# NBDsoftware/deep_cartograph

Measured on AMD Instinct MI355X. Metric: Deep-TICA training frames/sec on 10Mx512 feature matrix at 1/2/4/8 GPUs, higher is better.
Workload: dtype f32

## Files before the change

deep_cartograph_amd/csrc/gemm.h:

```cpp
#pragma once
#include <type_traits>
#include "common.h"
#include "handoff.h"

namespace dcv {

#ifdef DCV_STAMP
__device__ unsigned long long g_stamp[8 * 8192];
#define DCV_STAMP_AT(slot)                                                                      \
    do {                                                                                        \
        if (threadIdx.x == 0 && blockIdx.x < 8192 && blockIdx.z == 0)                           \
            g_stamp[blockIdx.x * 8 + (slot)] = __builtin_amdgcn_s_memtime();                   \
    } while (0)
#define DCV_STAMP_RT(slot)                                                                      \
    do {                                                                                        \
        if (threadIdx.x == 0 && blockIdx.x < 8192 && blockIdx.z == 0)                           \
            g_stamp[blockIdx.x * 8 + (slot)] = __builtin_amdgcn_s_memrealtime();               \
    } while (0)
#else
#define DCV_STAMP_AT(slot) do {} while (0)
#define DCV_STAMP_RT(slot) do {} while (0)
#endif

typedef float f32x16 __attribute__((ext_vector_type(16)));
// ... 43 lines not shown
    const float* p;
    int64_t ld;
    RowMap rows;
    const float* shift;
    int vec_ok;
    int planes = 0;
    int64_t pstride = 0;
};

struct GemmDims {
    int64_t M, N, K;
    int64_t k_chunk;
    int tiles_m, tiles_n;
    int xcd_remap;
    int wt;
    int tail_split = 0;
    float* tail_ws = nullptr;
    unsigned* tail_cnt = nullptr;
};

template <int WAVES_M_, int WAVES_N_, int FM_, int FN_, int KB_, int NBUF_ = 2, bool SPLIT_ = false, int PL_ = 0>
struct TileCfg {
    static constexpr int WAVES_M = WAVES_M_, WAVES_N = WAVES_N_, FM = FM_, FN = FN_, KB = KB_, NBUF = NBUF_;
    static constexpr bool SPLIT = SPLIT_;
    static constexpr int PL = PL_;
    static_assert(PL == 0 || SPLIT, "plane operands belong to the split flavour");
    static constexpr bool LS = (PL_ & 16) != 0;
    static constexpr int RAW_SZ = LS ? (WAVES_M_ * FM_ * 32 + WAVES_N_ * FN_ * 32) * KB_ : 0;
    static constexpr int A_SZ = (PL & 5) ? 3 * (WAVES_M_ * FM_ * 32) * (KB_ / 2) : (WAVES_M_ * FM_ * 32) * KB_;
    static constexpr int B_SZ = (PL & 10) ? 3 * (WAVES_N_ * FN_ * 32) * (KB_ / 2) : (WAVES_N_ * FN_ * 32) * KB_;
    static_assert(NBUF >= 2 && NBUF <= 8, "NBUF");
    static constexpr int TM = WAVES_M * FM * 32;
    static constexpr int TN = WAVES_N * FN * 32;
    static_assert(WAVES_M * WAVES_N == 4, "4 waves per workgroup");
    static_assert(KB == 16 || KB == 32, "KB");
};

template <int KB>
__device__ __forceinline__ int mmajor_off(int row, int chunk) {
    constexpr int CPR = KB / 4;
    constexpr int RPBR = 64 / KB;
    return row * KB + ((chunk ^ ((row / RPBR) % CPR)) << 2);
}

__device__ __forceinline__ void glds16(const float* gsrc, unsigned lds_wave_addr) {
    unsigned keep;
    asm volatile(
        "s_mov_b32 %0, m0\n\t"
        "s_mov_b32 m0, %2\n\t"
        "s_nop 0\n\t"
        "global_load_lds_dwordx4 %1, off\n\t"
        "s_mov_b32 m0, %0"
        : "=&s"(keep)
        : "v"(gsrc), "s"(lds_wave_addr)
        : "memory");
}
__device__ __forceinline__ unsigned lds_addr_uniform(const float* p) {
    const unsigned a = (unsigned)(uintptr_t)(__attribute__((address_space(3))) const float*)p;
    return __builtin_amdgcn_readfirstlane(a);
}

template <int PER>
__device__ __forceinline__ void glds16_batch(const float* base, const unsigned (&voff)[PER], unsigned lds0) {
    static_assert(PER == 1 || PER == 2 || PER == 4, "units per thread");
    unsigned keep;
    if constexpr (PER == 1) {
        asm volatile(
            "s_mov_b32 %0, m0\n\ts_nop 3\n\t"
// ... 296 lines not shown
__device__ __forceinline__ void vm_wait_younger(int64_t younger) {
    if constexpr (MAXY == 0) vm_wait<EXTRA>();
    else {
        if (younger >= MAXY) vm_wait<MAXY * GL + EXTRA>();
        else vm_wait_younger<MAXY - 1, GL, EXTRA>(younger);
    }
}

template <int MODE, class Cfg, int NB, bool VEC, bool GATHER, class Epi>
__device__ __forceinline__ void gemm_block(const Operand& A, const Operand& B, int64_t lag2, const GemmDims& d,
                                           int tile_m, int tile_n, int64_t k_begin, int64_t k_end, float* lds,
                                           Epi& epi, int tail_chunk = -1) {
    constexpr int TM = Cfg::TM, TN = Cfg::TN, KB = Cfg::KB, FM = Cfg::FM, FN = Cfg::FN;
    constexpr int A_SZ = Cfg::A_SZ, B_SZ = Cfg::B_SZ;
    constexpr int STAGE = A_SZ + NB * B_SZ;
    constexpr bool A_MM = (MODE == kNT || MODE == kNN);
    constexpr bool B_MM = (MODE == kNT);
    constexpr int PL = Cfg::PL;
    constexpr bool PRE = (PL & 3) != 0;
    constexpr bool PSA = (PL & 4) != 0, PSB = (PL & 8) != 0;
    constexpr bool PA = (PL & 5) != 0, PB = (PL & 10) != 0;
    constexpr bool LS = Cfg::LS;
    static_assert(!LS || (MODE == kNT && PSA && PSB && VEC && !GATHER && NB == 1), "split-from-LDS: NT products, both operands, 16-byte rows");
    static_assert(!PRE || (MODE == kNT && NB == 1 && VEC && Cfg::SPLIT), "plane operands: NT products of the split flavour");
    static_assert(!(PSA || PSB) || (!PRE && NB == 1 && Cfg::SPLIT), "split-at-store: split flavour, one B operand, no pre-split operand beside it");
    static_assert(!PSA || MODE == kNT || MODE == kNN, "split-at-store of A needs a contraction-contiguous A");
    static_assert(!PSB || MODE == kNT, "split-at-store of B needs a contraction-contiguous B");
    constexpr int KF = KB / 2;
    constexpr int KA = (PL & 1) ? KF : KB, KBB = (PL & 2) ? KF : KB;
    constexpr int NPA = (PL & 1) ? 3 : 1, NPB = (PL & 2) ? 3 : 1;
    const int t = threadIdx.x;
    const int lane = t & 63;
    const int wave = t >> 6;
    const int wm = (wave / Cfg::WAVES_N) * FM * 32;
    const int wn = (wave % Cfg::WAVES_N) * FN * 32;
    const int64_t m0 = (int64_t)tile_m * TM, n0 = (int64_t)tile_n * TN;
#ifdef DCV_ABL_SAMETILE
    const int64_t m0_ld = (int64_t)(tile_m % DCV_ABL_SAMETILE) * TM;
#else
    const int64_t m0_ld = m0;
#endif

    f32x16 acc[NB][FM][FN];
#pragma unroll
    for (int b = 0; b < NB; ++b)
#pragma unroll
        for (int i = 0; i < FM; ++i)
#pragma unroll
            for (int j = 0; j < FN; ++j)
#pragma unroll
                for (int e = 0; e < 16; ++e) acc[b][i][j][e] = 0.f;

    MMajorStage<TM, KA, VEC, GATHER> am;
    KMajorStage<TM, KB, VEC, GATHER> ak;
    MMajorStage<TN, KBB, VEC, GATHER> bm;
    KMajorStage<TN, KB, VEC, GATHER> bk[NB];
    if constexpr (A_MM) am.template init<PRE || LS>(A, m0, d.M, t);
    else ak.init(A, m0, d.M, t);
    if constexpr (B_MM) bm.template init<PRE || LS>(B, n0, d.N, t);
    else {
#pragma unroll
        for (int b = 0; b < NB; ++b) bk[b].init(B, n0, d.N, t);
    }

    auto resolve_stage = [&](int64_t k0) {
        if constexpr (!A_MM) ak.resolve(A, k0, k_end, 0, t);
        if constexpr (!B_MM) {
            bk[0].resolve(B, k0, k_end, 0, t);
// ... 292 lines not shown
        if constexpr (kASum) {
#pragma unroll
            for (int i = 0; i < FM; ++i) asum[i] += (f.a[i][0] + f.a[i][1]) + (f.a[i][2] + f.a[i][3]);
        }
    };
    auto mfma_step = [&](const Frags& f, int s) {
#pragma unroll
        for (int b = 0; b < NB; ++b)
#pragma unroll
            for (int i = 0; i < FM; ++i)
#pragma unroll
                for (int j = 0; j < FN; ++j)
                    acc[b][i][j] = __builtin_amdgcn_mfma_f32_32x32x2f32(f.a[i][s], f.b[b][j][s], acc[b][i][j], 0, 0, 0);
    };
    auto mfma_group = [&](const Frags& f) {
#pragma unroll
        for (int s = 0; s < 4; ++s)
#pragma unroll
            for (int b = 0; b < NB; ++b)
#pragma unroll
                for (int i = 0; i < FM; ++i)
#pragma unroll
                    for (int j = 0; j < FN; ++j)
                        acc[b][i][j] = __builtin_amdgcn_mfma_f32_32x32x2f32(f.a[i][s], f.b[b][j][s], acc[b][i][j], 0, 0, 0);
    };

    const int64_t nst = (k_end - k_begin + KB - 1) / KB;
    DCV_STAMP_AT(0);
#ifdef DCV_STAMP
    if (threadIdx.x == 0 && blockIdx.x < 8192 && blockIdx.z == 0)
        g_stamp[blockIdx.x * 8 + 7] = (unsigned long long)__builtin_amdgcn_s_getreg(63492) | ((unsigned long long)__builtin_amdgcn_s_getreg(63508) << 32);
#endif
    constexpr int G = KB / 8;
    auto compute_stage = [&](const float* cur) {
        const float* la = cur;
        const float* lb = cur + A_SZ;
        if constexpr (Cfg::SPLIT) {
#pragma unroll
            for (int s = 0; s < KB / 16; ++s) {
                Frags8 f;
                read_frags8(f, la, lb, s);
                mfma16(f);
            }
            return;
        }
#ifndef DCV_NO_FRAG_DBUF
        Frags f0, f1;
        read_frags(f0, la, lb, 0);
#pragma unroll
        for (int g = 0; g < G; g += 2) {
            if (g + 1 < G) read_frags(f1, la, lb, g + 1);
            add_asum(f0);
            mfma_group(f0);
            if (g + 1 < G) {
                if (g + 2 < G) read_frags(f0, la, lb, g + 2);
                add_asum(f1);
                mfma_group(f1);
            }
        }
#else
#pragma unroll
        for (int g = 0; g < G; ++g) {
            Frags f0;
            read_frags(f0, la, lb, g);
            add_asum(f0);
            mfma_group(f0);
        }
#endif
    };
// ... 62 lines not shown
    if (nfull > 0) {
        const int64_t nst = nfull;
        constexpr int NBUF = Cfg::NBUF;
        constexpr int GL = (A_MM ? NPA * MMajorStage<TM, KA, VEC, GATHER>::PER : KMajorStage<TM, KB, VEC, GATHER>::PER) +
                           NB * (B_MM ? NPB * MMajorStage<TN, KBB, VEC, GATHER>::PER : KMajorStage<TN, KB, VEC, GATHER>::PER);
        static_assert((NBUF - 2) * GL <= 63, "vmcnt range");
        static_assert(Cfg::SPLIT || G % 2 == 0, "fragment double buffer parity");
#pragma unroll
        for (int s = 0; s < NBUF - 1; ++s)
            if (s < nst) glds_stage(k_begin + s * KB, s);
        if constexpr (kSidePre) {
            static_assert((NBUF - 2) * GL + EPASS * ENQ <= 63, "vmcnt range");
            side_ready = epi.vec && (m0 + TM <= d.M) && (n0 + TN <= d.N);
            if constexpr (Epi::kMaskIn) side_ready = side_ready && epi.mask == nullptr;
            if (side_ready) {
                const int ec4 = t % EC4, er0 = t / EC4;
#pragma unroll
                for (int q = 0; q < EPASS * ENQ; ++q)
                    side_pre[q] = *reinterpret_cast<const float4*>(epi.side_ptr(m0 + er0 + q * ERPP, n0 + ec4 * 4));
                vm_wait_younger<NBUF - 2, GL, EPASS * ENQ>(nst - 1);
            } else {
                vm_wait_younger<NBUF - 2, GL>(nst - 1);
            }
        } else {
            vm_wait_younger<NBUF - 2, GL>(nst - 1);
        }
        __syncthreads();
#ifndef DCV_ABL_NOLOAD
        if (NBUF - 1 < nst) glds_stage(k_begin + (NBUF - 1) * KB, NBUF - 1);
#endif
        DCV_STAMP_AT(1);
        DCV_STAMP_RT(5);
        if constexpr (Cfg::SPLIT) {
            constexpr int S = KB / 16;
            Frags8 f0, f1;
#ifdef DCV_PIPE_SPLIT
            Planes pl0, pl1;
#endif
            read_frags8(f0, lds, lds + A_SZ, 0);
#ifdef DCV_PIPE_SPLIT
            if constexpr (S == 2) split_frags(f0, pl0);
#endif
            int cur_buf = 0;
            for (int64_t st = 0; st < nst; ++st) {
                const float* la = lds + cur_buf * STAGE;
                const float* lb = la + A_SZ;
                const int nxt_buf = cur_buf + 1 == NBUF ? 0 : cur_buf + 1;
#ifdef DCV_PIPE_SPLIT
                if constexpr (S == 2) {
                    constexpr int NMF = 6 * NB * FM * FN;
                    constexpr int NVA = 44 * (FM + NB * FN);
                    constexpr int VPM = (NVA + NMF - 1) / NMF;
                    read_frags8(f1, la, lb, 1);
                    mfma_planes(pl0, [](int) {});
                    split_frags(f1, pl1);
                    pin_planes(pl1);
#pragma unroll
                    for (int q = 0; q < NMF; ++q) {
                        __builtin_amdgcn_sched_group_barrier(0x008, 1, 0);
                        __builtin_amdgcn_sched_group_barrier(0x002, VPM, 0);
                    }
                    __builtin_amdgcn_sched_barrier(0);
                    vm_wait_younger<NBUF - 2, GL>(nst - 2 - st);
                    __syncthreads();
                    read_frags8(f0, lds + nxt_buf * STAGE, lds + nxt_buf * STAGE + A_SZ, 0);
                    const bool more = st + NBUF < nst;
                    const int64_t k_next = k_begin + (st + NBUF) * KB;
                    __builtin_amdgcn_sched_barrier(0);
                    if (more) glds_stage(k_next, cur_buf, 3);
                    __builtin_amdgcn_sched_barrier(0);
                    mfma_planes(pl1, [](int) {});
                    split_frags(f0, pl0);
// ... 5 lines not shown
                    }
                    __builtin_amdgcn_sched_barrier(0);
                } else
#endif
                if constexpr (S == 2) {
                    read_frags8(f1, la, lb, 1);
                    mfma16(f0);
                    Planes pl;
                    split_frags(f1, pl);
                    vm_wait_younger<NBUF - 2, GL>(nst - 2 - st);
#ifndef DCV_ABL_NOBARRIER
                    __syncthreads();
#endif
                    read_frags8(f0, lds + nxt_buf * STAGE, lds + nxt_buf * STAGE + A_SZ, 0);
                    const bool more = st + NBUF < nst;
                    const int64_t k_next = k_begin + (st + NBUF) * KB;
                    mfma_planes(pl, [&](int k) {
#ifndef DCV_ABL_NOLOAD
                        if (k == 0 || k == 2) {
                            __builtin_amdgcn_sched_barrier(0);
                            if (more) glds_stage(k_next, cur_buf, k == 0 ? 1 : 2);
                            __builtin_amdgcn_sched_barrier(0);
                        }
#endif
                    });
                } else {
                    vm_wait_younger<NBUF - 2, GL>(nst - 2 - st);
#ifndef DCV_ABL_NOBARRIER
                    __syncthreads();
#endif
#ifndef DCV_ABL_NOLOAD
                    if (st + NBUF < nst) glds_stage(k_begin + (st + NBUF) * KB, cur_buf);
#endif
                    read_frags8(f1, lds + nxt_buf * STAGE, lds + nxt_buf * STAGE + A_SZ, 0);
                    mfma16(f0);
                    f0 = f1;
                }
                cur_buf = nxt_buf;
            }
            __syncthreads();
        } else {
        Frags f0, f1;
        read_frags(f0, lds, lds + A_SZ, 0);
        int cur_buf = 0;
        for (int64_t st = 0; st < nst; ++st) {
            const float* la = lds + cur_buf * STAGE;
            const float* lb = la + A_SZ;
            const int nxt_buf = cur_buf + 1 == NBUF ? 0 : cur_buf + 1;
#pragma unroll
            for (int g = 0; g < G; g += 2) {
                read_frags(f1, la, lb, g + 1);
                __builtin_amdgcn_sched_barrier(0);
                pin_frags(f0);
                if (dma_sub) sub_frags(f0);
                add_asum(f0);
                mfma_group(f0);
                __builtin_amdgcn_sched_barrier(0);
                if (g + 2 < G) {
                    read_frags(f0, la, lb, g + 2);
                    __builtin_amdgcn_sched_barrier(0);
                    pin_frags(f1);
                    if (dma_sub) sub_frags(f1);
                    add_asum(f1);
                    mfma_group(f1);
                    __builtin_amdgcn_sched_barrier(0);
                } else {
                    vm_wait_younger<NBUF - 2, GL>(nst - 2 - st);
// ... 18 lines not shown
                    __builtin_amdgcn_sched_barrier(0);
                    mfma_step(f1, 2);
                    __builtin_amdgcn_sched_barrier(0);
                    read_frags(f0, lds + nxt_buf * STAGE, lds + nxt_buf * STAGE + A_SZ, 0);
                    __builtin_amdgcn_sched_barrier(0);
                    mfma_step(f1, 3);
                    __builtin_amdgcn_sched_barrier(0);
                }
            }
            cur_buf = nxt_buf;
        }
        __syncthreads();
        }
    } else {
        DCV_STAMP_AT(1);
        DCV_STAMP_RT(5);
    }
    const int64_t k_rem = k_begin + nfull * KB;
    const int64_t nrem = (PRE || LS) ? 0 : (k_end - k_rem + KB - 1) / KB;
    if (nrem > 0) {
        resolve_stage(k_rem);
        load_stage(k_rem);
        if (nrem > 1) resolve_stage(k_rem + KB);
        store_stage(lds);
        __syncthreads();
        for (int64_t st = 0; st < nrem; ++st) {
            const float* cur = lds + (st & 1) * STAGE;
            float* nxt = lds + ((st + 1) & 1) * STAGE;
            const bool more = st + 1 < nrem;
            if (more) {
                load_stage(k_rem + (st + 1) * KB);
                if (st + 2 < nrem) resolve_stage(k_rem + (st + 2) * KB);
            }
            if (MODE == kTN || m0 + wm < d.M) compute_stage(cur);
            if (more) store_stage(nxt);
            __syncthreads();
        }
    }
    if constexpr (MODE != kTN && NB == 1) {
        if (tail_chunk >= 0) {
            constexpr int NACC = FM * FN * 16;
            const int S = d.tail_split;
            float* ws = d.tail_ws + (int64_t)tile_n * S * NACC * 256;
            float* mine = ws + (int64_t)tail_chunk * NACC * 256 + t;
#pragma unroll
            for (int i = 0; i < FM; ++i)
#pragma unroll
                for (int j = 0; j < FN; ++j)
#pragma unroll
                    for (int e = 0; e < 16; ++e) handoff_store(mine + ((i * FN + j) * 16 + e) * 256, acc[0][i][j][e]);
            const bool last = handoff_arrive_last(d.tail_cnt + tile_n, (unsigned)S, reinterpret_cast<unsigned*>(lds));
            __syncthreads();
            if (!last) return;
#pragma unroll
            for (int i = 0; i < FM; ++i)
#pragma unroll
                for (int j = 0; j < FN; ++j)
#pragma unroll
                    for (int e = 0; e < 16; ++e) acc[0][i][j][e] = 0.f;
            for (int c = 0; c < S; ++c) {
                const float* part = ws + (int64_t)c * NACC * 256 + t;
#pragma unroll
                for (int i = 0; i < FM; ++i)
#pragma unroll
                    for (int j = 0; j < FN; ++j)
#pragma unroll
                        for (int e = 0; e < 16; ++e) acc[0][i][j][e] += handoff_load(part + ((i * FN + j) * 16 + e) * 256);
            }
        }
    }
#ifdef DCV_ABL_NOEPI
    {
        float sink = 0.f;
#pragma unroll
        for (int b = 0; b < NB; ++b)
#pragma unroll
            for (int i = 0; i < FM; ++i)
#pragma unroll
                for (int j = 0; j < FN; ++j)
#pragma unroll
                    for (int e = 0; e < 16; ++e) sink += acc[b][i][j][e];
        if (sink != 12345.678f) return;
    }
#endif

    DCV_STAMP_AT(2);
    DCV_STAMP_RT(6);
    static_assert(!Epi::kHead || kStaged, "the fused narrow layer needs the staged epilogue");
    if constexpr (kStaged) {
        float* tile = lds;
        constexpr int C4 = TN / 4;
        constexpr int RPP = 256 / C4;
        constexpr int NQ = RP / RPP;
        const int c4 = t % C4, r0 = t / C4;
        const int64_t col = n0 + c4 * 4;
        const int64_t left = d.N - col;
        const int nvalid = left >= 4 ? 4 : (left > 0 ? (int)left : 0);
        const bool fast = epi.vec && (m0 + TM <= d.M) && (n0 + TN <= d.N);
        const float4 cc = nvalid > 0 ? epi.colconst(col, nvalid) : make_float4(0.f, 0.f, 0.f, 0.f);
        constexpr int EQ = NQ < 8 ? NQ : 8;
        static_assert(NQ % EQ == 0, "epilogue chunking");
        float4 cs = make_float4(0.f, 0.f, 0.f, 0.f);
#pragma unroll
        for (int ep = 0; ep < EPASS; ++ep) {
            if (ep > 0) __syncthreads();
            if (wm / RP == ep) {
#pragma unroll
                for (int i = 0; i < FM; ++i)
#pragma unroll
                    for (int j = 0; j < FN; ++j) {
                        const int c = wn + j * 32 + (lane & 31);
                        const int rb = wm - ep * RP + i * 32 + 4 * (lane >> 5);
#pragma unroll
                        for (int e = 0; e < 16; ++e) tile[(rb + (e & 3) + 8 * (e >> 2)) * TN + c] = acc[0][i][j][e];
                    }
            }
            __syncthreads();
            if (ep == 0) DCV_STAMP_AT(3);
            const int64_t mbase = m0 + ep * RP;
#pragma unroll
            for (int qc = 0; qc < NQ; qc += EQ) {
                float4 v[EQ], side[Epi::kSide ? EQ : 1];
// ... 115 lines not shown
```

deep_cartograph_amd/csrc/gemm.hip:

```cpp
#include <type_traits>
#include "gemm_kernels.h"

using namespace dcv;

namespace dcv {
int gemm_nn_store(const Operand& A, const Operand& B, int64_t M, int64_t N, int64_t K, const EpiStore& epi, hipStream_t s) {
    return launch_gemm<kNN, EpiStore>(A, B, M, N, K, 0, epi, s);
}
}

extern "C" int dcv_gemm_f32(int32_t mode, const float* A_d, int64_t lda, const float* B_d, int64_t ldb, float* C_d,
                            int64_t ldc, int64_t M, int64_t N, int64_t K, void* stream) {
    DCV_REQUIRE(A_d && B_d && C_d && M > 0 && N > 0 && K > 0, "dcv_gemm_f32: bad arguments");
    hipStream_t s = as_stream(stream);
    const Operand A = make_operand(A_d, lda, 0);
    const Operand B = make_operand(B_d, ldb, 0);
    EpiStore epi{C_d, ldc, quad_ok(C_d, ldc)};
    switch (mode) {
        case kNT: return launch_gemm<kNT, EpiStore>(A, B, M, N, K, 0, epi, s);
        case kNN: return gemm_nn_store(A, B, M, N, K, epi, s);
        case kTN: return launch_gemm<kTN, EpiStore>(A, B, M, N, K, 0, epi, s);
        default: set_error("dcv_gemm_f32: mode %d", mode); return DCV_EINVAL;
    }
}

extern "C" int dcv_gemm_tn_split(const float* A_d, int64_t lda, const float* B_d, int64_t ldb, float* slab_d, int64_t slab_cap,
                                 int64_t M, int64_t N, int64_t K, int64_t k_chunk, void* stream) {
    DCV_REQUIRE(A_d && B_d && slab_d && M > 0 && N > 0 && K > 0 && k_chunk > 0 && slab_cap > 0, "dcv_gemm_tn_split: bad arguments");
    const Operand A = make_operand(A_d, lda, 0);
    const Operand B = make_operand(B_d, ldb, 0);
    EpiSlab epi{slab_d, M, N, 1, 0, quad_ok(slab_d, N), slab_cap};
    return gemm_tn_slab(A, B, M, N, K, k_chunk, epi, as_stream(stream));
}
```

deep_cartograph_amd/csrc/gemm_kernels.h:

```cpp
#pragma once
#include <type_traits>
#include <stdlib.h>
#include <hip/hip_ext.h>
#include "gemm.h"

namespace dcv {

constexpr float kSoftplus0 = 0.6931471824645996f;
__device__ __forceinline__ float act_fwd(int act, float z) {
    switch (act) {
        case DCV_ACT_LEAKY_RELU: return z > 0.f ? z : 0.01f * z;
        case DCV_ACT_RELU: return z > 0.f ? z : 0.f;
        case DCV_ACT_TANH: return tanhf(z);
        case DCV_ACT_ELU: return z > 0.f ? z : expm1f(z);
        case DCV_ACT_SOFTPLUS: return z > 20.f ? z : log1pf(expf(z));
        case DCV_ACT_SHIFTED_SOFTPLUS: return (z > 20.f ? z : log1pf(expf(z))) - kSoftplus0;
        case DCV_ACT_CUSTOM_SIGMOID: return 1.f / (1.f + expf(-3.f * z));
        default: return z;
    }
}
__device__ __forceinline__ float act_grad_from_out(int act, float h) {
    switch (act) {
        case DCV_ACT_LEAKY_RELU: return h > 0.f ? 1.f : 0.01f;
        case DCV_ACT_RELU: return h > 0.f ? 1.f : 0.f;
// ... 323 lines not shown
        gemm_block<kNN, Cfg2, 1, true, false, EpiActGrad>(A2, B2, 0, d2, bm.tile_m, bm.tile_n, bm.k_begin, bm.k_end, lds_f, e2, bm.tail_chunk);
    }
}

struct GroupShift {
    int64_t a_rows = 0;
    int64_t a_floats = 0;
    int64_t out_rows = 0;
    int64_t tail_floats = 0;
    int tail_tickets = 0;
};
template <class Cfg, bool VEC, bool GATHER, class Epi>
__global__ __launch_bounds__(256, 2) void gemm_group_kernel(Operand A, Operand B, GemmDims d, Epi epi, GroupShift g) {
    extern __shared__ __attribute__((aligned(16))) float lds_f[];
    const int64_t j = blockIdx.y;
    A.p += j * g.a_floats;
    if (A.rows.idx != nullptr) A.rows.idx += j * g.a_rows;
    else A.rows.row0 += j * g.a_rows;
    epi.shift_rows(j * g.out_rows);
    if (d.tail_split > 0) {
        d.tail_ws += j * g.tail_floats;
        d.tail_cnt += j * g.tail_tickets;
    }
    const BlockMap bm = map_block<kNT>(d, (int)blockIdx.x);
    gemm_block<kNT, Cfg, 1, VEC, GATHER, Epi>(A, B, 0, d, bm.tile_m, bm.tile_n, bm.k_begin, bm.k_end, lds_f, epi, bm.tail_chunk);
}

template <bool S> using CfgBigT = TileCfg<2, 2, 2, 2, 32, 2, S>;
template <bool S> using CfgHalfMT = TileCfg<2, 2, 1, 2, 32, 2, S>;
template <bool S> using CfgQuarterT = TileCfg<2, 2, 1, 1, 32, 2, S>;
template <bool S> using CfgNarrowNT = TileCfg<4, 1, 1, 1, 32, 2, S>;
template <bool S> using CfgNarrowMT = TileCfg<1, 4, 1, 1, 32, 2, S>;
template <bool S> using CfgCovT = TileCfg<2, 2, 2, 2, 16, 2, S>;
#ifdef DCV_BIGCFG
using CfgBig = DCV_BIGCFG;
#else
using CfgBig = CfgBigT<false>;
#endif

template <int MODE, class Cfg, int NB, bool VEC, bool GATHER, class Epi>
static int launch_gemm_vec(const Operand& A, const Operand& B, int64_t lag2, const GemmDims& d, int64_t splits,
                           const Epi& epi, hipStream_t s) {
#ifdef DCV_FORCE_LDS
    constexpr size_t lds = DCV_FORCE_LDS;
#else
    constexpr size_t lds = gemm_lds_bytes<Cfg, NB>();
#endif
    auto kern = gemm_kernel<MODE, Cfg, NB, VEC, GATHER, Epi>;
    if (lds > 64 * 1024) {
        static bool attr_set = false;
        if (!attr_set) {
            DCV_CHECK_HIP(hipFuncSetAttribute(reinterpret_cast<const void*>(kern), hipFuncAttributeMaxDynamicSharedMemorySize, (int)lds));
            attr_set = true;
        }
    }
    const int64_t blocks = d.tail_split > 0 ? (int64_t)(d.tiles_m - 1 + d.tail_split) * d.tiles_n : (int64_t)d.tiles_m * d.tiles_n;
    if (g_launch_ev.start != nullptr) {
        const LaunchEvents ev = g_launch_ev;
        g_launch_ev = LaunchEvents{};
        g_launch_taken = ev.start;
        hipExtLaunchKernelGGL(kern, dim3((unsigned)blocks, 1, (unsigned)splits), dim3(256), (uint32_t)lds, s, ev.start, ev.stop, 0u, A, B, lag2, d, epi);
    } else {
        hipLaunchKernelGGL(kern, dim3((unsigned)blocks, 1, (unsigned)splits), dim3(256), lds, s, A, B, lag2, d, epi);
    }
    DCV_CHECK_LAUNCH();
    return DCV_OK;
// ... 171 lines not shown
            }
        }
    }
#endif
#ifdef DCV_PS_EXPERIMENT
    if constexpr (S && MODE == kNT && !Epi::kHead) {
        static const bool ls_on = [] { const char* e = getenv("DCV_LS"); return e && e[0] == '1'; }();
        if (ls_on && pick == kPickQuarter) {
            const int rc = launch_gemm_ls<TileCfg<2, 2, 1, 1, 32, 2, true, 28>, Epi>(A, B, M, N, K, epi, s, tiles_m_out, tw);
            if (rc != 1) return rc;
        }
    }
#endif
    switch (pick) {
        case kPickNarrowN: return launch_gemm_cfg<MODE, CfgNarrowNT<S>, 1, Epi>(A, B, 0, M, N, K, k_chunk, epi, s, tiles_m_out, tw);
        case kPickNarrowM: return launch_gemm_cfg<MODE, CfgNarrowMT<S>, 1, Epi>(A, B, 0, M, N, K, k_chunk, epi, s, tiles_m_out, tw);
        case kPickHalfM: return launch_gemm_cfg<MODE, CfgHalfMT<S>, 1, Epi>(A, B, 0, M, N, K, k_chunk, epi, s, tiles_m_out, tw);
        case kPickQuarter:
            if constexpr (!Epi::kHead) return launch_gemm_cfg<MODE, CfgQuarterT<S>, 1, Epi>(A, B, 0, M, N, K, k_chunk, epi, s, tiles_m_out, tw);
            else return launch_gemm_cfg<MODE, CfgHalfMT<S>, 1, Epi>(A, B, 0, M, N, K, k_chunk, epi, s, tiles_m_out, tw);
        default: return launch_gemm_cfg<MODE, Big, 1, Epi>(A, B, 0, M, N, K, k_chunk, epi, s, tiles_m_out, tw);
    }
}

template <int MODE, class Epi>
static int launch_gemm(const Operand& A, const Operand& B, int64_t M, int64_t N, int64_t K, int64_t k_chunk,
                       const Epi& epi, hipStream_t s, int* tiles_m_out = nullptr, const TailWs* tw = nullptr) {
#ifdef DCV_BIGCFG
    return launch_gemm_mode<MODE, false, Epi>(A, B, M, N, K, k_chunk, epi, s, tiles_m_out, tw);
#else
    if (gemm_split()) return launch_gemm_mode<MODE, true, Epi>(A, B, M, N, K, k_chunk, epi, s, tiles_m_out, tw);
    return launch_gemm_mode<MODE, false, Epi>(A, B, M, N, K, k_chunk, epi, s, tiles_m_out, tw);
#endif
}

template <bool S, bool HEAD, class F>
static int with_cfg(CfgPick pick, F&& f) {
    switch (pick) {
        case kPickNarrowN: return f(CfgNarrowNT<S>{});
        case kPickNarrowM: return f(CfgNarrowMT<S>{});
        case kPickHalfM: return f(CfgHalfMT<S>{});
        case kPickQuarter:
            if constexpr (!HEAD) return f(CfgQuarterT<S>{});
            else return f(CfgHalfMT<S>{});
        default: return f(CfgBigT<S>{});
    }
}
inline bool group_retile_enabled() {
    static const bool on = [] { const char* e = getenv("DCV_EVAL_GROUP_TILES"); return !(e && e[0] == '0'); }();
    return on;
}
template <bool S, class Epi>
static int launch_gemm_group_mode(const Operand& A, const Operand& B, int64_t M, int64_t N, int64_t K, const Epi& epi, const GroupShift& g,
                                  int members, const TailWs* tw, hipStream_t s) {
    constexpr bool HEAD = Epi::kHead;
    DCV_REQUIRE(members >= 1 && members < 65536, "gemm: %d members in a grouped launch", members);
    const CfgPick pick1 = pick_cfg<kNT, HEAD>(M, N, K, 0);
    GemmPlan single;
    int64_t tm1 = 0;
    int rc = with_cfg<S, HEAD>(pick1, [&](auto c) {
        using C1 = decltype(c);
        tm1 = C1::TM;
        return prepare_gemm<kNT, C1, 1, Epi>(A, B, M, N, K, 0, epi, nullptr, tw, &single);
    });
    if (rc) return rc;
    if (!single.vec) return 1;
// ... 19 lines not shown
            if (r) return r;
            if (!pl.vec) return 1;
            if (single.d.tail_split > 0) {
                constexpr int64_t TM2 = C2::TM;
                const int64_t S1 = single.d.tail_split;
                if (M % TM2 == 0 || (M / TM2) * TM2 != (M / tm1) * tm1 || pl.d.tiles_m < 2 || K % C2::KB != 0) return 1;
                if (pl.d.tiles_n > tw->max_tiles_n || (int64_t)pl.d.tiles_n * S1 * C2::FM * C2::FN * 16 * 256 > tw->cap) return 1;
                pl.d.tail_split = (int)S1;
                pl.d.k_chunk = single.d.k_chunk;
                pl.d.tail_ws = single.d.tail_ws;
                pl.d.tail_cnt = single.d.tail_cnt;
                pl.d.xcd_remap = xcd_remap_enabled() && (pl.d.tiles_m - 1) % 8 == 0 && pl.d.tiles_n > 1;
            }
            return go(c, pl);
        });
        if (rc != 1) return rc;
    }
    return with_cfg<S, HEAD>(pick1, [&](auto c) { return go(c, single); });
}
template <class Epi>
static int launch_gemm_group(const Operand& A, const Operand& B, int64_t M, int64_t N, int64_t K, const Epi& epi, const GroupShift& g, int members,
                             const TailWs* tw, hipStream_t s) {
    if (gemm_split()) return launch_gemm_group_mode<true, Epi>(A, B, M, N, K, epi, g, members, tw, s);
    return launch_gemm_group_mode<false, Epi>(A, B, M, N, K, epi, g, members, tw, s);
}

int gemm_nt_bias_act(const Operand& A, const Operand& B, int64_t M, int64_t N, int64_t K, const EpiBiasAct& epi, hipStream_t s, const TailWs* tw);
int gemm_nt_head4(const Operand& A, const Operand& B, int64_t M, int64_t N, int64_t K, const EpiBiasActHead<4>& epi, hipStream_t s, const TailWs* tw);
int gemm_nt_head8(const Operand& A, const Operand& B, int64_t M, int64_t N, int64_t K, const EpiBiasActHead<8>& epi, hipStream_t s, const TailWs* tw);
int gemm_nt_bias_act_group(const Operand& A, const Operand& B, int64_t M, int64_t N, int64_t K, const EpiBiasAct& epi, const GroupShift& g, int members,
                           const TailWs* tw, hipStream_t s);
int gemm_nt_head4_group(const Operand& A, const Operand& B, int64_t M, int64_t N, int64_t K, const EpiBiasActHead<4>& epi, const GroupShift& g, int members,
                        const TailWs* tw, hipStream_t s);
int gemm_tn_slab(const Operand& A, const Operand& B, int64_t M, int64_t N, int64_t K, int64_t k_chunk, const EpiSlab& epi, hipStream_t s);
int gemm_nn_act_grad(const Operand& A, const Operand& B, int64_t M, int64_t N, int64_t K, const EpiActGrad& epi, hipStream_t s,
                     int* tiles_m_out, const TailWs* tw);
int gemm_nn_store(const Operand& A, const Operand& B, int64_t M, int64_t N, int64_t K, const EpiStore& epi, hipStream_t s);

int launch_wgrad_dgrad(const Operand& A1, const Operand& B1, int64_t M1, int64_t N1, int64_t K1, int64_t k_chunk1, const EpiSlab& e1,
                       const Operand& A2, const Operand& B2, int64_t M2, int64_t N2, int64_t K2, const EpiActGrad& e2, int* tiles_m_out2,
                       const TailWs* tw, hipStream_t s);

__host__ __device__ inline int64_t planes_kp(int64_t cols) { return (cols + 31) / 32 * 32; }
__host__ __device__ inline int64_t planes_ld(int64_t cols) { return 3 * planes_kp(cols) / 2; }
__host__ __device__ inline int64_t planes_pstride(int64_t cols) { return planes_kp(cols) / 2; }
inline size_t planes_bytes(int64_t rows, int64_t cols) { return (size_t)rows * (size_t)planes_ld(cols) * sizeof(float); }
template <bool TRANS>
__global__ __launch_bounds__(256) void split_planes_kernel(const float* __restrict__ src, int64_t ld, int64_t rows, int64_t cols,
                                                           float* __restrict__ dst, int64_t rows_out) {
    const int64_t orows = TRANS ? cols : rows, ocols = TRANS ? rows : cols;
    const int64_t kp8 = planes_kp(ocols) / 8, ldp = planes_ld(ocols), ps = planes_pstride(ocols);
    const int64_t total = rows_out * kp8;
    for (int64_t i = (int64_t)blockIdx.x * 256 + threadIdx.x; i < total; i += (int64_t)gridDim.x * 256) {
        const int64_t r = i / kp8, g = i - r * kp8;
        float x[8];
#pragma unroll
        for (int e = 0; e < 8; ++e) {
            const int64_t k = 8 * g + e;
            x[e] = (r < orows && k < ocols) ? (TRANS ? src[k * ld + r] : src[r * ld + k]) : 0.f;
        }
        u32x4 p1, p2, p3;
        split3(x, p1, p2, p3);
        float* o = dst + r * ldp + g * 4;
        *reinterpret_cast<u32x4*>(o) = p1;
        *reinterpret_cast<u32x4*>(o + ps) = p2;
        *reinterpret_cast<u32x4*>(o + 2 * ps) = p3;
    }
// ... 90 lines not shown
```

deep_cartograph_amd/csrc/inst_wgrad.hip:

```cpp
#include "gemm_kernels.h"

namespace dcv {

int gemm_tn_slab(const Operand& A, const Operand& B, int64_t M, int64_t N, int64_t K, int64_t k_chunk, const EpiSlab& epi, hipStream_t s) {
    return launch_gemm<kTN, EpiSlab>(A, B, M, N, K, k_chunk, epi, s);
}

}
```

deep_cartograph_amd/csrc/mlp.hip:

```cpp
#include "mlp_state.h"
#include "tica_head.h"
#include <new>
#include <math.h>

using namespace dcv;

namespace dcv {

constexpr int kColsumRows = 32;
constexpr int kSseRows = 16;
constexpr int kStatBlockRows = 128;

__global__ __launch_bounds__(256) void colsum_kernel(const float* __restrict__ Z, int64_t rows, int n, int64_t ld,
                                                     float* __restrict__ part) {
    __shared__ float red[256];
    const int64_t r0 = (int64_t)blockIdx.x * kColsumRows;
    const int64_t r1 = r0 + kColsumRows < rows ? r0 + kColsumRows : rows;
    const int t = threadIdx.x;
    const int cols = n < 256 ? n : 256;
    const int groups = 256 / cols;
    const int c_in = t % cols, g = t / cols;
    for (int c0 = 0; c0 < n; c0 += cols) {
        const int c = c0 + c_in;
        float s = 0.f;
// ... 2135 lines not shown
            prof_mark(m, l, 1, 1, s);
            Operand Bd = make_operand(m->params + p.w_off, p.in, p.in);
            EpiActGrad eg{dz_nxt, m->ld_dz, m->vae_z, m->ld_z, DCV_ACT_NONE, hd.bpart, p.in, quad_ok(dz_nxt, m->ld_dz) && quad_ok(m->vae_z, m->ld_z)};
            int dblocks = 0;
            prof_mark(m, l, 2, 0, s);
            rc = gemm_nn_act_grad(A, Bd, R, p.in, p.out, eg, s, &dblocks, &m->tail);
            if (rc) return rc;
            hipLaunchKernelGGL(vae_sample_backward_kernel, dim3((unsigned)cdiv(R, kVaeRows)), dim3(kVaeRows), 0, s, (const float*)hd.H, hd.ldh, R,
                               m->vae_d, m->eps_cur, dz_nxt, m->ld_dz, (float)(m->kl_beta / (double)global_batch));
            DCV_CHECK_LAUNCH();
            bblocks = (int)cdiv(R, kColsumRows);
            hipLaunchKernelGGL(colsum_kernel, dim3(bblocks), dim3(256), 0, s, (const float*)dz_nxt, R, hd.out, m->ld_dz, hd.bpart);
            DCV_CHECK_LAUNCH();
            prof_mark(m, l, 2, 1, s);
            float* tmp = dz_cur;
            dz_cur = dz_nxt;
            dz_nxt = tmp;
            continue;
        }
        Operand A = make_operand(dz_cur, m->ld_dz, p.out);
        Operand B = l == 0 ? make_operand(Xn_d, ld, p.in, rm) : make_operand(layer_out(m, l - 1), m->layers[l - 1].ldh, p.in);
        EpiSlab epi{p.slab, p.out, p.in, 1, 0, quad_ok(p.slab, p.in), p.max_splits};
        ReduceDesc& rd = ra.l[l];
        rd.slab = p.slab;
        rd.bpart = p.bpart;
        rd.w_off = p.w_off;
        rd.b_off = p.b_off;
        rd.w_count = (int64_t)p.out * p.in;
        rd.out = p.out;
        rd.splits = (int)splits;
        rd.bblocks = bblocks;
        if (l == 0) {
            prof_mark(m, l, 1, 0, s);
            int rc = gemm_tn_slab(A, B, p.out, p.in, R, kc, epi, s);
            if (rc) return rc;
            prof_mark(m, l, 1, 1, s);
            continue;
        }
        LayerPlan& q = m->layers[l - 1];
        Operand Ad = make_operand(dz_cur, m->ld_dz, p.out);
        Operand Bd = make_operand(m->params + p.w_off, p.in, p.in);
        EpiActGrad eg{dz_nxt, m->ld_dz, q.H, q.ldh, q.act, q.bpart, q.out, quad_ok(dz_nxt, m->ld_dz) && quad_ok(q.H, q.ldh)};
        if (q.mask && q.mask_rows == R) {
            eg.mask = q.mask;
            eg.slope = q.act == DCV_ACT_LEAKY_RELU ? 0.01f : 0.f;
        }
        eg.drop = drop_cfg(m, l - 1);
        eg.hscale = drop_hscale(m, l - 1);
        if (q.bn) {
            eg.act = DCV_ACT_NONE;
            eg.mask = nullptr;
            eg.drop = kNoDrop;
            eg.hscale = 1.f;
        }
        prof_mark(m, l, 1, 0, s);
        prof_mark(m, l, 2, 0, s);
        int rc = launch_wgrad_dgrad(A, B, p.out, p.in, R, kc, epi, Ad, Bd, R, p.in, p.out, eg, &bblocks, &m->tail, s);
        if (rc < 0) return rc;
        if (rc == 1) {
            rc = gemm_tn_slab(A, B, p.out, p.in, R, kc, epi, s);
            if (rc) return rc;
            prof_mark(m, l, 1, 1, s);
            prof_mark(m, l, 2, 0, s);
            rc = gemm_nn_act_grad(Ad, Bd, R, p.in, p.out, eg, s, &bblocks, &m->tail);
            if (rc) return rc;
            prof_mark(m, l, 2, 1, s);
        } else {
// ... 677 lines not shown
```

Measured before the change: 80.31 million.

## Add wave-K split TN GEMM path for first-layer weight gradient

Adds a wave-K tile layout in which the four waves of a workgroup each take a different 16-deep slice of the contraction. Each wave writes its partial tile to LDS, and the epilogue sums the partials before storing. The first-layer weight-gradient GEMM uses this path when the picker would choose the quarter config, split mode is on and no row gather is used. The aim is more parallelism and less per-wave tile overhead on the small-output, long-K wgrad product, at the cost of an extra LDS reduction and a barrier in the epilogue.

```diff
diff --git a/deep_cartograph_amd/csrc/gemm.h b/deep_cartograph_amd/csrc/gemm.h
--- a/deep_cartograph_amd/csrc/gemm.h
+++ b/deep_cartograph_amd/csrc/gemm.h
@@ -99,8 +99,10 @@
     static_assert(NBUF >= 2 && NBUF <= 8, "NBUF");
     static constexpr int TM = WAVES_M * FM * 32;
     static constexpr int TN = WAVES_N * FN * 32;
-    static_assert(WAVES_M * WAVES_N == 4, "4 waves per workgroup");
-    static_assert(KB == 16 || KB == 32, "KB");
+    static constexpr int WAVES_K = 4 / (WAVES_M * WAVES_N);
+    static_assert(WAVES_M * WAVES_N * WAVES_K == 4, "4 waves per workgroup");
+    static_assert(KB == 16 || KB == 32 || (KB == 64 && WAVES_K == 4), "KB");
+    static_assert(WAVES_K == 1 || (SPLIT && PL == 0 && KB == 16 * WAVES_K), "wave-K layouts: split flavour, one 16-deep step per wave and stage");
 };
 
 template <int KB>
@@ -463,8 +465,13 @@
     const int t = threadIdx.x;
     const int lane = t & 63;
     const int wave = t >> 6;
-    const int wm = (wave / Cfg::WAVES_N) * FM * 32;
-    const int wn = (wave % Cfg::WAVES_N) * FN * 32;
+    constexpr int WK = Cfg::WAVES_K;
+    static_assert(WK == 1 || (MODE == kTN && NB == 1 && !Epi::kColSum && !Epi::kSide && !Epi::kHead && !Epi::kMaskOut && !Epi::kMaskIn && !Epi::kDrop),
+                  "wave-K layouts: contraction-split TN products with a plain-store epilogue");
+    const int wk = WK > 1 ? __builtin_amdgcn_readfirstlane(wave / (Cfg::WAVES_M * Cfg::WAVES_N)) : 0;
+    const int wmn = WK > 1 ? wave % (Cfg::WAVES_M * Cfg::WAVES_N) : wave;
+    const int wm = (wmn / Cfg::WAVES_N) * FM * 32;
+    const int wn = (wmn % Cfg::WAVES_N) * FN * 32;
     const int64_t m0 = (int64_t)tile_m * TM, n0 = (int64_t)tile_n * TN;
 #ifdef DCV_ABL_SAMETILE
     const int64_t m0_ld = (int64_t)(tile_m % DCV_ABL_SAMETILE) * TM;
@@ -823,9 +830,17 @@
         g_stamp[blockIdx.x * 8 + 7] = (unsigned long long)__builtin_amdgcn_s_getreg(63492) | ((unsigned long long)__builtin_amdgcn_s_getreg(63508) << 32);
 #endif
     constexpr int G = KB / 8;
-    auto compute_stage = [&](const float* cur) {
+    auto compute_stage = [&](const float* cur, int64_t kleft = Cfg::KB) {
         const float* la = cur;
         const float* lb = cur + A_SZ;
+        if constexpr (WK > 1) {
+            if (16 * wk < kleft) {
+                Frags8 f;
+                read_frags8(f, la, lb, wk);
+                mfma16(f);
+            }
+            return;
+        }
         if constexpr (Cfg::SPLIT) {
 #pragma unroll
             for (int s = 0; s < KB / 16; ++s) {
@@ -954,12 +969,13 @@
         DCV_STAMP_AT(1);
         DCV_STAMP_RT(5);
         if constexpr (Cfg::SPLIT) {
-            constexpr int S = KB / 16;
+            constexpr int S = WK > 1 ? 1 : KB / 16;
+            const int s0 = WK > 1 ? wk : 0;
             Frags8 f0, f1;
 #ifdef DCV_PIPE_SPLIT
             Planes pl0, pl1;
 #endif
-            read_frags8(f0, lds, lds + A_SZ, 0);
+            read_frags8(f0, lds, lds + A_SZ, s0);
 #ifdef DCV_PIPE_SPLIT
             if constexpr (S == 2) split_frags(f0, pl0);
 #endif
@@ -1031,7 +1047,7 @@
 #ifndef DCV_ABL_NOLOAD
                     if (st + NBUF < nst) glds_stage(k_begin + (st + NBUF) * KB, cur_buf);
 #endif
-                    read_frags8(f1, lds + nxt_buf * STAGE, lds + nxt_buf * STAGE + A_SZ, 0);
+                    read_frags8(f1, lds + nxt_buf * STAGE, lds + nxt_buf * STAGE + A_SZ, s0);
                     mfma16(f0);
                     f0 = f1;
                 }
@@ -1116,7 +1132,7 @@
                 load_stage(k_rem + (st + 1) * KB);
                 if (st + 2 < nrem) resolve_stage(k_rem + (st + 2) * KB);
             }
-            if (MODE == kTN || m0 + wm < d.M) compute_stage(cur);
+            if (MODE == kTN || m0 + wm < d.M) compute_stage(cur, k_end - (k_rem + st * KB));
             if (more) store_stage(nxt);
             __syncthreads();
         }
@@ -1171,7 +1187,56 @@
     DCV_STAMP_AT(2);
     DCV_STAMP_RT(6);
     static_assert(!Epi::kHead || kStaged, "the fused narrow layer needs the staged epilogue");
-    if constexpr (kStaged) {
+    if constexpr (WK > 1) {
+        constexpr int C4 = TN / 4;
+        constexpr int RPP = 256 / C4;
+        constexpr int NQ = TM / RPP;
+        static_assert(WK * TM * TN <= LDSF, "wave-K layouts: the stage buffers must hold one tile image per contraction wave");
+        static_assert(256 % C4 == 0 && TM % RPP == 0, "wave-K epilogue geometry");
+        float* part = lds + wk * (TM * TN);
+#pragma unroll
+        for (int i = 0; i < FM; ++i)
+#pragma unroll
+            for (int j = 0; j < FN; ++j) {
+                const int c = wn + j * 32 + (lane & 31);
+                const int rb = wm + i * 32 + 4 * (lane >> 5);
+#pragma unroll
+                for (int e = 0; e < 16; ++e) part[(rb + (e & 3) + 8 * (e >> 2)) * TN + c] = acc[0][i][j][e];
+            }
+        __syncthreads();
+        DCV_STAMP_AT(3);
+        const int c4 = t % C4, r0 = t / C4;
+        const int64_t col = n0 + c4 * 4;
+        const int64_t left = d.N - col;
+        const int nvalid = left >= 4 ? 4 : (left > 0 ? (int)left : 0);
+        const bool fast = epi.vec && (m0 + TM <= d.M) && (n0 + TN <= d.N);
+        float4 v[NQ];
+#pragma unroll
+        for (int q = 0; q < NQ; ++q) {
+            const float* src = lds + (r0 + q * RPP) * TN + c4 * 4;
+            v[q] = *reinterpret_cast<const float4*>(src);
+#pragma unroll
+            for (int w = 1; w < WK; ++w) {
+                const float4 u = *reinterpret_cast<const float4*>(src + w * (TM * TN));
+                v[q].x += u.x; v[q].y += u.y; v[q].z += u.z; v[q].w += u.w;
+            }
+        }
+#pragma unroll
+        for (int q = 0; q < NQ; ++q) {
+            const int64_t row = m0 + r0 + q * RPP;
+            if (fast) {
+                if (d.wt) {
+                    hv4f hv = {v[q].x, v[q].y, v[q].z, v[q].w};
+                    handoff_store16(epi.out_ptr(0, row, col), hv);
+                } else {
+                    *reinterpret_cast<float4*>(epi.out_ptr(0, row, col)) = v[q];
+                }
+            } else if (row < d.M && nvalid > 0) {
+                store_quad(epi.out_ptr(0, row, col), v[q], nvalid, epi.vec);
+            }
+        }
+        DCV_STAMP_AT(4);
+    } else if constexpr (kStaged) {
         float* tile = lds;
         constexpr int C4 = TN / 4;
         constexpr int RPP = 256 / C4;
diff --git a/deep_cartograph_amd/csrc/gemm.hip b/deep_cartograph_amd/csrc/gemm.hip
--- a/deep_cartograph_amd/csrc/gemm.hip
+++ b/deep_cartograph_amd/csrc/gemm.hip
@@ -30,5 +30,5 @@
     const Operand A = make_operand(A_d, lda, 0);
     const Operand B = make_operand(B_d, ldb, 0);
     EpiSlab epi{slab_d, M, N, 1, 0, quad_ok(slab_d, N), slab_cap};
-    return gemm_tn_slab(A, B, M, N, K, k_chunk, epi, as_stream(stream));
+    return gemm_tn_slab(A, B, M, N, K, k_chunk, epi, as_stream(stream), true);
 }
diff --git a/deep_cartograph_amd/csrc/gemm_kernels.h b/deep_cartograph_amd/csrc/gemm_kernels.h
--- a/deep_cartograph_amd/csrc/gemm_kernels.h
+++ b/deep_cartograph_amd/csrc/gemm_kernels.h
@@ -379,6 +379,10 @@
 template <bool S> using CfgNarrowNT = TileCfg<4, 1, 1, 1, 32, 2, S>;
 template <bool S> using CfgNarrowMT = TileCfg<1, 4, 1, 1, 32, 2, S>;
 template <bool S> using CfgCovT = TileCfg<2, 2, 2, 2, 16, 2, S>;
+using CfgWaveK4 = TileCfg<1, 1, 2, 2, 64, 2, true>;
+using CfgWaveK2Q = TileCfg<1, 2, 2, 1, 32, 2, true>;
+using CfgWaveK2N = TileCfg<1, 2, 2, 2, 32, 3, true>;
+using CfgWaveK2M = TileCfg<2, 1, 2, 2, 32, 3, true>;
 #ifdef DCV_BIGCFG
 using CfgBig = DCV_BIGCFG;
 #else
@@ -616,6 +620,23 @@
     if (gemm_split()) return launch_gemm_mode<MODE, true, Epi>(A, B, M, N, K, k_chunk, epi, s, tiles_m_out, tw);
     return launch_gemm_mode<MODE, false, Epi>(A, B, M, N, K, k_chunk, epi, s, tiles_m_out, tw);
 #endif
+}
+
+inline bool wgrad_wavek_enabled() {
+    static const bool on = [] { const char* e = getenv("DCV_WGRAD_WAVEK"); return !(e && e[0] == '0'); }();
+    return on;
+}
+using CfgWgradWaveK = CfgWaveK4;
+inline bool wgrad_takes_wavek(bool allow, int64_t M, int64_t N, int64_t K, int64_t k_chunk) {
+    return allow && gemm_split() && wgrad_wavek_enabled() && pick_cfg<kTN, false>(M, N, K, k_chunk) == kPickQuarter;
+}
+template <class Cfg, class Epi>
+static int launch_gemm_wavek(const Operand& A, const Operand& B, int64_t M, int64_t N, int64_t K, int64_t k_chunk, const Epi& epi, hipStream_t s) {
+    GemmPlan pl;
+    const int rc = prepare_gemm<kTN, Cfg, 1, Epi>(A, B, M, N, K, k_chunk, epi, nullptr, nullptr, &pl);
+    if (rc) return rc;
+    if (!pl.vec || pl.gather) return 1;
+    return launch_gemm_vec<kTN, Cfg, 1, true, false, Epi>(A, B, 0, pl.d, pl.splits, epi, s);
 }
 
 template <bool S, bool HEAD, class F>
@@ -701,7 +722,7 @@
                            const TailWs* tw, hipStream_t s);
 int gemm_nt_head4_group(const Operand& A, const Operand& B, int64_t M, int64_t N, int64_t K, const EpiBiasActHead<4>& epi, const GroupShift& g, int members,
                         const TailWs* tw, hipStream_t s);
-int gemm_tn_slab(const Operand& A, const Operand& B, int64_t M, int64_t N, int64_t K, int64_t k_chunk, const EpiSlab& epi, hipStream_t s);
+int gemm_tn_slab(const Operand& A, const Operand& B, int64_t M, int64_t N, int64_t K, int64_t k_chunk, const EpiSlab& epi, hipStream_t s, bool wavek = false);
 int gemm_nn_act_grad(const Operand& A, const Operand& B, int64_t M, int64_t N, int64_t K, const EpiActGrad& epi, hipStream_t s,
                      int* tiles_m_out, const TailWs* tw);
 int gemm_nn_store(const Operand& A, const Operand& B, int64_t M, int64_t N, int64_t K, const EpiStore& epi, hipStream_t s);
diff --git a/deep_cartograph_amd/csrc/inst_wgrad.hip b/deep_cartograph_amd/csrc/inst_wgrad.hip
--- a/deep_cartograph_amd/csrc/inst_wgrad.hip
+++ b/deep_cartograph_amd/csrc/inst_wgrad.hip
@@ -2,7 +2,11 @@
 
 namespace dcv {
 
-int gemm_tn_slab(const Operand& A, const Operand& B, int64_t M, int64_t N, int64_t K, int64_t k_chunk, const EpiSlab& epi, hipStream_t s) {
+int gemm_tn_slab(const Operand& A, const Operand& B, int64_t M, int64_t N, int64_t K, int64_t k_chunk, const EpiSlab& epi, hipStream_t s, bool wavek) {
+    if (wgrad_takes_wavek(wavek, M, N, K, k_chunk)) {
+        const int rc = launch_gemm_wavek<CfgWgradWaveK, EpiSlab>(A, B, M, N, K, k_chunk, epi, s);
+        if (rc != 1) return rc;
+    }
     return launch_gemm<kTN, EpiSlab>(A, B, M, N, K, k_chunk, epi, s);
 }
 
diff --git a/deep_cartograph_amd/csrc/mlp.hip b/deep_cartograph_amd/csrc/mlp.hip
--- a/deep_cartograph_amd/csrc/mlp.hip
+++ b/deep_cartograph_amd/csrc/mlp.hip
@@ -2191,7 +2191,7 @@
         rd.bblocks = bblocks;
         if (l == 0) {
             prof_mark(m, l, 1, 0, s);
-            int rc = gemm_tn_slab(A, B, p.out, p.in, R, kc, epi, s);
+            int rc = gemm_tn_slab(A, B, p.out, p.in, R, kc, epi, s, idx_d == nullptr);
             if (rc) return rc;
             prof_mark(m, l, 1, 1, s);
             continue;
```

Result: no change. 80.58 million, median of 2 (+0.3%).
